# PSeitz/lz4_flex

Measured on AMD Instinct MI355X. Metric: MiB/s compress+decompress round trip, 1 GiB of 64 KiB JSON blocks per GPU (LZ4 block format), higher is better.
Workload: dtype u8

## Files before the change

lz4_flex_amd/csrc/capi.cpp:

```cpp
#include <hip/hip_runtime.h>

#include <algorithm>
#include <cstdio>
#include <cstdlib>
#include <cstring>
#include <mutex>
#include <new>
#include <string>
#include <vector>

#include "../../include/lz4flex_amd.h"
#include "lz4_batch_entry.h"
#include "lz4_ctx.h"
#include "lz4_device.h"
#include "lz4_plan_common.h"

using namespace lz4flex_dev;

static thread_local std::string g_last_error;
static thread_local int g_last_hip = 0;

static int hip_fail(hipError_t e, const char* what) {
    g_last_hip = (int)e;
    g_last_error = std::string(what) + ": " + hipGetErrorString(e);
// ... 278 lines not shown

extern "C" {

const char* lz4flex_version(void) { return "lz4flex-amd 0.3.0 (gfx950)"; }
#ifndef LZ4FLEX_BUILD_ID
#define LZ4FLEX_BUILD_ID "unstamped"
#endif
const char* lz4flex_build_id(void) { return LZ4FLEX_BUILD_ID; }
const char* lz4flex_last_error(void) { return g_last_error.c_str(); }

int lz4flex_device_count(void) {
    int n = 0;
    if (hipGetDeviceCount(&n) != hipSuccess) return 0;
    return n;
}

int lz4flex_ctx_create(lz4flex_ctx** out, int device) {
    if (!out) return -LZ4FLEX_E_INVALID_ARG;
    *out = nullptr;
    int n = 0;
    hipError_t e = hipGetDeviceCount(&n);
    if (e != hipSuccess || n <= 0) {
        g_last_error = "no HIP device available: the MI355X kernels are the only codec in this library";
        return -LZ4FLEX_E_NO_DEVICE;
    }
    if (device < 0) HIP_TRY(hipGetDevice(&device));
    if (device >= n) return -LZ4FLEX_E_INVALID_ARG;
    lz4flex_ctx* c = new (std::nothrow) lz4flex_ctx();
    if (!c) return -LZ4FLEX_E_NOMEM;
    c->device = device;
    c->packed_tile = (int)PACKED_SCAN_TILE;
    if (const char* e = getenv("LZ4FLEX_COMPRESS_MODE")) c->comp_mode = (!strcmp(e, "exact") || !strcmp(e, "1")) ? 1 : (!strcmp(e, "high") || !strcmp(e, "2")) ? 2 : 0;
    if (const char* e = getenv("LZ4FLEX_HIGH_PARSE")) c->comp_parse = (!strcmp(e, "optimal") || !strcmp(e, "1")) ? 1 : 0;
    if (const char* e = getenv("LZ4FLEX_HIGH_DICT")) c->comp_high_dict = !strcmp(e, "1") ? 1 : 0;
    if (const char* e = getenv("LZ4FLEX_HIGH_LINKED")) c->comp_high_linked = !strcmp(e, "1") ? 1 : 0;
    if (const char* e = getenv("LZ4FLEX_SLIDING_WINDOW")) {
        if (!strcmp(e, "0") || !strcmp(e, "1") || !strcmp(e, "2")) c->comp_sliding = e[0] - '0';
        else { g_last_error = "LZ4FLEX_SLIDING_WINDOW must be 0, 1 or 2"; delete c; return -LZ4FLEX_E_INVALID_ARG; }
    }
#ifdef LZ4FLEX_ALL_VARIANTS
    if (const char* e = getenv("LZ4FLEX_COMPRESS_VARIANT")) { const int v = atoi(e); if (v == 1 || v == 3) c->comp_variant = v; }
#endif
    if (const char* e = getenv("LZ4FLEX_DECOMPRESS_VARIANT")) { const int v = atoi(e); if (v == 0 || v == 1 || (v >= 4 && v <= 12 && v != 9)) c->dec_variant = v; }
    {
        DeviceGuard guard(device);
        e = guard.err;
        if (e == hipSuccess) e = hipStreamCreateWithFlags(&c->stream, hipStreamNonBlocking);
        if (e == hipSuccess) {
            int cus = 0;
            e = hipDeviceGetAttribute(&cus, hipDeviceAttributeMultiprocessorCount, device);
            if (e == hipSuccess) {
                c->wave_wgs = 2 * cus;
                e = hipMalloc(&c->wave_ws, compress_wave_workspace_bytes(c->wave_wgs));
            }
        }
        if (e == hipSuccess) e = c->wave.create();
        if (e == hipSuccess) e = hipMalloc((void**)&c->chain_ws, 4u * CHAIN_MAX_BLOCKS);
        if (e == hipSuccess) e = c->chain.create();
        if (e == hipSuccess) e = c->plan.create();
        if (e == hipSuccess) e = c->pcd.create();
        if (e == hipSuccess) e = hipMalloc((void**)&c->pcd_ws, decompress_pcd_pair_ws_bytes());
    }
    if (e != hipSuccess) {
        const int rc = hip_fail(e, "ctx_create");
        lz4flex_ctx_destroy(c);
        return e == hipErrorOutOfMemory ? -LZ4FLEX_E_NOMEM : rc;
    }
    *out = c;
    return 0;
}

void lz4flex_ctx_destroy(lz4flex_ctx* c) {
    if (!c) return;
    c->arena.free();
    if (c->wave_ws) (void)hipFree(c->wave_ws);
    c->wave.destroy();
    if (c->chain_ws) (void)hipFree(c->chain_ws);
    c->chain.destroy();
    if (c->plan_ws) (void)hipFree(c->plan_ws);
    c->plan.destroy();
    if (c->pcd_ws) (void)hipFree(c->pcd_ws);
    c->pcd.destroy();
    if (c->wave_prof) (void)hipFree(c->wave_prof);
    for (void* p : c->many_ws) if (p) (void)hipFree(p);
    c->pin.free();
    c->pay.free();
    if (c->stream) (void)hipStreamDestroy(c->stream);
    delete c;
}

#ifdef LZ4FLEX_TOOLS
int lz4flex_debug_wave_prof(lz4flex_ctx* c, int enable, unsigned long long* vals) {
    if (!c) return -LZ4FLEX_E_INVALID_ARG;
    if (vals && c->wave_prof) {
        HIP_TRY(hipDeviceSynchronize());
        HIP_TRY(hipMemcpy(vals, c->wave_prof, 256, hipMemcpyDeviceToHost));
    }
    if (enable) {
        if (!c->wave_prof) HIP_TRY(hipMalloc((void**)&c->wave_prof, 256));
        HIP_TRY(hipMemset(c->wave_prof, 0, 256));
    } else if (c->wave_prof) {
        (void)hipFree(c->wave_prof);
        c->wave_prof = nullptr;
    }
    return 0;
}
// ... 46 lines not shown
     }, false},
    {"compress_lanes", &lz4flex_ctx::comp_lanes, [](int v) { return v == 8 || v == 16; }, false},
    {"size_scan_serial", &lz4flex_ctx::size_serial, is_flag, false},
    {"filter_bytewise", &lz4flex_ctx::filter_bytewise, is_flag, false},
    {"fit_serial", &lz4flex_ctx::fit_serial, is_flag, false},
    {"compress_shared_dict", &lz4flex_ctx::comp_shared, is_flag, false},
    {"decompress_shared_dict", &lz4flex_ctx::dec_shared, is_flag, false},
    {"decompress_partial", &lz4flex_ctx::dec_partial, is_flag, false},
    {"frame_range_pass_bytes", &lz4flex_ctx::range_pass_bytes, [](int v) { return v >= 1; }, false},
    {"frame_range_checksums", &lz4flex_ctx::range_checksums, is_flag, false},
    {"packed_scan_tile", &lz4flex_ctx::packed_tile, read_only, false},
    {"compress_workgroups", &lz4flex_ctx::wave_wgs, read_only, false},
    {"debug_chain_giveup", &lz4flex_ctx::chain_giveup, is_count, true},
    {"debug_exact_dict_piece", &lz4flex_ctx::exact_dict_piece, is_count, true},
    {"debug_fail_next_batch", &lz4flex_ctx::fail_next_batch, is_count, true},
    {"debug_fit_first_pass", &lz4flex_ctx::fit_first_pass, is_flag, true},
};
const Setting* find_setting(const char* key) {
    for (const Setting& s : SETTINGS) if (!strcmp(key, s.key)) return &s;
    return nullptr;
}

bool key_allowed(const char* key) {
    if (strncmp(key, "debug_", 6) != 0) return true;
    const char* e = getenv("LZ4FLEX_TEST_HOOKS");
    return e && !strcmp(e, "1");
}

int list_index(const char* index) { return index[0] < '0' || index[0] > '9' ? -1 : atoi(index); }

int shared_dict_items(lz4flex_ctx* c) {
    if (!c->shared_counted || !c->wave_ws) return 0;
    DeviceGuard guard(c->device);
    HIP_TRY(guard.err);
    uint32_t v = 0;
    hipError_t e = hipDeviceSynchronize();
    if (e == hipSuccess) e = hipMemcpy(&v, compress_wave_shared_counter(c->wave_ws, c->wave_wgs), 4, hipMemcpyDeviceToHost);
    if (e != hipSuccess) return hip_fail(e, "debug_shared_dict_items");
    return (int)std::min<uint32_t>(v, 0x7FFFFFFFu);
}

int dict_set_items(lz4flex_ctx* c) {
    std::lock_guard<std::mutex> lock(g_sets_mu);
    if (!c->set_counted || std::find(g_live_sets.begin(), g_live_sets.end(), c->set_counted) == g_live_sets.end()) return 0;
    DeviceGuard guard(c->device);
    HIP_TRY(guard.err);
    uint32_t v = 0;
    hipError_t e = hipDeviceSynchronize();
    if (e == hipSuccess) e = hipMemcpy(&v, c->set_counted->counter, 4, hipMemcpyDeviceToHost);
    if (e != hipSuccess) return hip_fail(e, "debug_dict_set_items");
    return (int)std::min<uint32_t>(v, 0x7FFFFFFFu);
}

}

extern "C" {

int lz4flex_set_tuning(lz4flex_ctx* c, const char* key, int value) {
    if (!key) return -LZ4FLEX_E_INVALID_ARG;
    const Setting* st = find_setting(key);
    if (!st || !key_allowed(key)) return -LZ4FLEX_E_INVALID_ARG;
    if (!c) { const int rc = default_ctx(&c); if (rc) return rc; }
    if (!st->takes(value)) return -LZ4FLEX_E_INVALID_ARG;
    c->*(st->field) = value;
    return 0;
}

int lz4flex_get_tuning(lz4flex_ctx* c, const char* key) {
    if (!key) return -LZ4FLEX_E_INVALID_ARG;
    if (!strncmp(key, "dispatch_threshold_", 19)) {
        const int i = list_index(key + 19);
        return i >= 0 && i < (int)(sizeof DISPATCH_THRESHOLDS / sizeof DISPATCH_THRESHOLDS[0]) ? (int)DISPATCH_THRESHOLDS[i] : -LZ4FLEX_E_INVALID_ARG;
    }
    if (!strncmp(key, "decoder_config_", 15)) {
        const int v = decoder_config(list_index(key + 15), TOOLS_BUILD);
        return v >= 0 ? v : -LZ4FLEX_E_INVALID_ARG;
    }
    const bool set_items = !strcmp(key, "debug_dict_set_items");
    const bool items = set_items || !strcmp(key, "debug_shared_dict_items");
    const Setting* st = items ? nullptr : find_setting(key);
    if ((!items && !st) || !key_allowed(key)) return -LZ4FLEX_E_INVALID_ARG;
    if (!c) { const int rc = default_ctx(&c); if (rc) return rc; }
    if (items) return set_items ? dict_set_items(c) : shared_dict_items(c);
    return st->set_only ? -LZ4FLEX_E_INVALID_ARG : c->*(st->field);
}

int lz4flex_abi_version(void) { return 8; }

size_t lz4flex_get_maximum_output_size(size_t input_len) {
    return 16 + 4 + (size_t)((uint64_t)input_len * 110 / 100);
}

}

namespace {

struct Span {
    uint64_t lo = ~0ull, hi = 0;
    void add(uint64_t off, uint64_t len) { lo = std::min<uint64_t>(lo, off); hi = std::max<uint64_t>(hi, off + len); }
    Span closed() const { return lo > hi ? Span{0, 0} : *this; }
    size_t bytes() const { return (size_t)(hi - lo); }
};
Span span_of(const uint64_t* off, const uint32_t* len, uint32_t n) {
    Span s;
    for (uint32_t i = 0; i < n; i++) s.add(off[i], len[i]);
    return s.closed();
}

bool host_big(const uint32_t* len, uint32_t n, bool compress) {
    const uint32_t limit = compress ? 65536u : 131072u;
    bool big = false;
    for (uint32_t i = 0; i < n; i++) big |= len[i] > limit;
    return big;
}

void copy_results(const BatchCall& b, const uint32_t* r_len, const int32_t* r_st, const uint64_t* r_det) {
    memcpy(b.out_len, r_len, 4ull * b.n);
    memcpy(b.status, r_st, 4ull * b.n);
    if (!b.detail) return;
    if (b.compress) memset(b.detail, 0, 16ull * b.n);
    else memcpy(b.detail, r_det, 16ull * b.n);
}

template <class SrcOff>
void scatter_good(uint8_t* out_base, const uint64_t* out_off, const uint32_t* len, const int32_t* st, uint32_t n, const uint8_t* src, SrcOff src_off,
                  uint64_t limit = ~0ull) {
    for (uint32_t i = 0; i < n; i++)
        if ((!st || st[i] == 0) && len[i] && (uint64_t)src_off(i) + len[i] <= limit) memcpy(out_base + out_off[i], src + src_off(i), len[i]);
}

}

static constexpr uint32_t SMALL_BATCH_BLOCKS = 8u;
static constexpr size_t SMALL_BATCH_BYTES = 4u << 20;
static int run_host_small(lz4flex_ctx* c, const BatchCall& b) {
    const uint32_t n = b.n;
// ... 1418 lines not shown
```

lz4_flex_amd/csrc/lz4_compress_wave.hip:

```cpp
#include <hip/hip_runtime.h>
#include <stdint.h>

#include "lz4_device.h"

namespace lz4flex_dev {
namespace wave {

typedef __attribute__((address_space(3))) uint8_t lds_u8;
typedef __attribute__((address_space(3))) uint16_t lds_u16;
typedef __attribute__((address_space(3))) uint32_t lds_u32;
typedef uint32_t u32x4 __attribute__((ext_vector_type(4)));
typedef __attribute__((address_space(1))) uint8_t g_u8;
typedef __attribute__((address_space(1))) u32x4 g_u32x4;
typedef uint32_t u32x2 __attribute__((ext_vector_type(2)));
typedef __attribute__((address_space(1))) u32x2 g_u32x2;
typedef __attribute__((address_space(1))) uint32_t g_u32;
typedef __attribute__((address_space(1))) int32_t g_i32;

constexpr uint32_t WINDOW = 65536u;
#ifndef LZ4W_WORKERS
#define LZ4W_WORKERS 11
#endif
constexpr uint32_t WORKERS = LZ4W_WORKERS;
constexpr uint32_t GROUPS = WINDOW / 512u;
// ... 5 lines not shown
    if (WORKERS == 8u) {
        constexpr uint32_t lo[9] = {0u, 16u, 33u, 50u, 67u, 82u, 98u, 113u, 128u};
        return 512u * lo[w < 8u ? w : 8u];
    }
    return 512u * ((GROUPS * w) / WORKERS);
}
__host__ __device__ constexpr uint32_t seg_longest() {
    uint32_t m = 0u;
    for (uint32_t w = 0u; w < WORKERS; ++w) m = seg_lo(w + 1u) - seg_lo(w) > m ? seg_lo(w + 1u) - seg_lo(w) : m;
    return m;
}
constexpr uint32_t SEG = seg_longest();
constexpr uint32_t HIST = WINDOW / 2u;
__device__ __forceinline__ uint32_t seg_start(uint32_t j, uint32_t skip, uint32_t send) {
    if (send == 0u) return seg_lo(j) > skip ? seg_lo(j) : skip;
    if (j == 0u) return skip;
    if (j >= WORKERS) return send;
    const uint32_t span = send > skip ? send - skip : 0u;
    const uint32_t v = (skip + span * (seg_lo(j) / 512u) / 128u) & ~511u;
    return v > skip ? v : skip;
}

constexpr uint32_t CAP = 1024u;
constexpr uint32_t SKIPD = 64u;
constexpr uint32_t CARRY_SLOTS = 16u;
constexpr uint32_t CARRY_DWORDS = CARRY_SLOTS * 16u;
constexpr uint32_t CARRY_SPINS = 1u << 18;
constexpr uint32_t LONGK = 84u;
constexpr uint32_t NEARP = 20u;
constexpr uint32_t LONGN = 8u;
constexpr uint32_t HBITS = 12u;
constexpr uint32_t THREADS = 64u * (WORKERS + 1u);
#ifndef LZ4W_RING_SLOTS
#define LZ4W_RING_SLOTS 1
#endif
constexpr uint32_t RING_SLOTS = LZ4W_RING_SLOTS;
constexpr uint32_t TMP_OFF = 16u;
constexpr uint32_t CMP_OFF = TMP_OFF + 256u;
constexpr uint32_t WORKER_LDS = CMP_OFF + 256u;
constexpr uint32_t CHUNK = 1024u;
constexpr uint32_t CHUNK_SLOT = CHUNK + 16u;
constexpr uint32_t IDX_DEPTH = 4u;
constexpr uint32_t L_WIN = 0u;
constexpr uint32_t L_TAB = WINDOW + 64u;
constexpr uint32_t L_STG = L_TAB + (2u << HBITS);
constexpr uint32_t L_RING = L_STG + WORKERS * WORKER_LDS;
constexpr uint32_t L_META = L_RING + RING_SLOTS * CHUNK_SLOT;
constexpr uint32_t M_RUN = 5u * WORKERS + 8u;
constexpr uint32_t M_TICKET = M_RUN + 2u;
constexpr uint32_t M_REC = M_TICKET + 1u;
constexpr uint32_t REC_SEG = 7u;
constexpr uint32_t REC_UNI = REC_SEG * WORKERS;
constexpr uint32_t REC_WORDS = REC_UNI + 18u;
constexpr uint32_t META_WORDS = M_REC + 2u * REC_WORDS;
constexpr uint32_t LDS_BYTES = L_META + ((META_WORDS * 4u + 63u) & ~63u);
static_assert(LDS_BYTES <= 81920u, "two workgroups per CU");
static_assert(WORKERS >= 1u && WORKERS <= 15u && seg_lo(WORKERS) == WINDOW, "segments tile the window");
constexpr uint32_t SLOT_BYTES = 2u * WINDOW;
constexpr uint32_t BODY_STRIDE = (SEG + SEG / 128u + 255u) / 256u * 256u + 256u;
constexpr uint32_t BODY_SET = WORKERS * BODY_STRIDE;
constexpr uint32_t WS_BYTES = 2u * SLOT_BYTES + 2u * BODY_SET;
static_assert(WS_BYTES % 256u == 0u, "workspace slots stay 256 B aligned");
constexpr uint32_t STAGE_BYTES = WINDOW + 256u;
constexpr uint32_t STAGE_READ = WINDOW + 64u;

struct SegMeta {
    uint32_t has;
    uint32_t first_lit;
    uint32_t first_ml;
    uint32_t trail;
    uint32_t body_len;
};
struct BlkCarry { uint32_t out_pos, pend; };

__device__ __forceinline__ uint32_t dpp_wave_shr1(uint32_t v, uint32_t lane0) {
    return (uint32_t)__builtin_amdgcn_update_dpp((int)lane0, (int)v, 0x138, 0xf, 0xf, false);
}
__device__ __forceinline__ uint32_t dpp_wave_shl1(uint32_t v, uint32_t lane63) {
    return (uint32_t)__builtin_amdgcn_update_dpp((int)lane63, (int)v, 0x130, 0xf, 0xf, false);
}
#define LZ4W_DPP(v, ctrl, rmask) ((uint32_t)__builtin_amdgcn_update_dpp(0, (int)(v), (ctrl), (rmask), 0xf, false))
__device__ __forceinline__ uint32_t wave_incl_max(uint32_t v) {
    uint32_t t;
    t = LZ4W_DPP(v, 0x111, 0xf); v = v > t ? v : t;
    t = LZ4W_DPP(v, 0x112, 0xf); v = v > t ? v : t;
    t = LZ4W_DPP(v, 0x114, 0xf); v = v > t ? v : t;
    t = LZ4W_DPP(v, 0x118, 0xf); v = v > t ? v : t;
    t = LZ4W_DPP(v, 0x142, 0xa); v = v > t ? v : t;
    t = LZ4W_DPP(v, 0x143, 0xc); v = v > t ? v : t;
    return v;
}
__device__ __forceinline__ uint32_t wave_incl_add(uint32_t v) {
    v += LZ4W_DPP(v, 0x111, 0xf);
    v += LZ4W_DPP(v, 0x112, 0xf);
    v += LZ4W_DPP(v, 0x114, 0xf);
    v += LZ4W_DPP(v, 0x118, 0xf);
    v += LZ4W_DPP(v, 0x142, 0xa);
    v += LZ4W_DPP(v, 0x143, 0xc);
    return v;
}
__device__ __forceinline__ uint32_t rdlane(uint32_t v, uint32_t l) { return (uint32_t)__builtin_amdgcn_readlane((int)v, (int)l); }
__device__ __forceinline__ uint32_t uni(uint32_t v) { return (uint32_t)__builtin_amdgcn_readfirstlane((int)v); }
__device__ __forceinline__ uint64_t ld64l(const lds_u8* p) { uint64_t v; __builtin_memcpy(&v, (const void*)p, 8); return v; }
__device__ __forceinline__ uint32_t umin3(uint32_t a, uint32_t b, uint32_t c) { const uint32_t t = a < b ? a : b; return t < c ? t : c; }
__device__ __forceinline__ uint32_t ctz64(uint64_t x) { return (uint32_t)__builtin_ctzll(x); }
__device__ __forceinline__ uint32_t len_ext_bytes(uint32_t v) { return v >= 15u ? (v - 15u) / 255u + 1u : 0u; }

// ... 184 lines not shown
#endif
#define LZ4W_ONE_CHUNK(N, CC, J)                                                                    \
        {                                                                                           \
            lds_u8* sl = lds + L_RING + ((J) & (RING_SLOTS - 1u)) * CHUNK_SLOT;                                    \
            chunk_wait<N>(q[J]);                                                                    \
            __builtin_memcpy((void*)(sl + 16u * lane), &q[J].main, 16);                             \
            __builtin_memcpy((void*)(sl + CHUNK), &q[J].extra, 4);    \
            const uint32_t cn = (CC) + IDX_DEPTH;                                                   \
            chunk_issue(q[J], gwin, cn < last ? cn : last, lane);                                   \
            index_chunk<true>(sl + lane4, tab, cand_lane, (CC), act_n, lane);                       \
        }
        static_assert(IDX_DEPTH == 4u, "the wait counts below are for four chunks in flight");
        uint32_t c = c0;
        if (n_main - c0 >= IDX_DEPTH) {
            LZ4W_ONE_CHUNK(6, c0, 0)
            LZ4W_ONE_CHUNK(10, c0 + 1u, 1)
            LZ4W_ONE_CHUNK(14, c0 + 2u, 2)
            LZ4W_ONE_CHUNK(18, c0 + 3u, 3)
            c = c0 + IDX_DEPTH;
        }
        for (; c + IDX_DEPTH <= n_main; c += IDX_DEPTH) {
            LZ4W_ONE_CHUNK(22, c, 0)
            LZ4W_ONE_CHUNK(22, c + 1u, 1)
            LZ4W_ONE_CHUNK(22, c + 2u, 2)
            LZ4W_ONE_CHUNK(22, c + 3u, 3)
        }
#undef LZ4W_ONE_CHUNK
        chunk_wait<0>(q[0]); chunk_wait<0>(q[1]); chunk_wait<0>(q[2]); chunk_wait<0>(q[3]);
        for (uint32_t j = 0; c < n_main; ++c, ++j) {
            lds_u8* sl = lds + L_RING + (j & (RING_SLOTS - 1u)) * CHUNK_SLOT;
            const ChunkRegs r = j == 0u ? q[0] : (j == 1u ? q[1] : q[2]);
            __builtin_memcpy((void*)(sl + 16u * lane), &r.main, 16);
            __builtin_memcpy((void*)(sl + CHUNK), &r.extra, 4);
            index_chunk<true>(sl + lane4, tab, cand_lane, c, act_n, lane);
        }
    }
    for (uint32_t c = n_main; c < nchunks; ++c) {
        lds_u8* sl = lds + L_RING;
        const uint32_t base = c * CHUNK;
        for (uint32_t i = lane; i < (CHUNK + 16u) / 16u; i += 64u) {
            const uint32_t o = base + 16u * i;
            u32x4 v = {0u, 0u, 0u, 0u};
            if (o + 16u <= rd_n) __builtin_memcpy(&v, (const void*)(gwin + o), 16);
            __builtin_memcpy((void*)(sl + 16u * i), &v, 16);
        }
        const uint32_t part = rd_n > base ? ((rd_n - base) & ~15u) : 0u;
        if (part < CHUNK + 16u && lane < 16u) {
            const uint32_t o = base + part + lane;
            if (part + lane < CHUNK + 16u) sl[part + lane] = o < rd_n ? gwin[o] : (uint8_t)0;
        }
        index_chunk<false>(sl + lane4, tab, cand_lane, c, act_n, lane);
    }
    return 0u;
}

__device__ __forceinline__ u32x4 tail16(const g_u8* __restrict__ tail, uint32_t o, uint32_t h) {
    u32x4 v = {0u, 0u, 0u, 0u};
    if (o + 16u <= h) __builtin_memcpy(&v, (const void*)(tail + o), 16);
    else if (o < h) {
        uint32_t wd[4] = {0u, 0u, 0u, 0u};
#pragma unroll
        for (uint32_t k = 0; k < 16u; ++k)
            if (o + k < h) wd[k >> 2] |= (uint32_t)tail[o + k] << (8u * (k & 3u));
        v = u32x4{wd[0], wd[1], wd[2], wd[3]};
    }
    return v;
}
__device__ __forceinline__ void digest_body(const uint8_t* __restrict__ dict, uint32_t dict_len, uint8_t* __restrict__ digest,
                                            uint8_t* __restrict__ cand_scratch, lds_u8* lds) {
    const uint32_t lane = threadIdx.x;
    const uint32_t h = dict_len < HIST ? dict_len : HIST, hs = digest_hs(h);
    const g_u8* __restrict__ tail = (const g_u8*)dict + (dict_len - h);
    g_u8* __restrict__ dg = (g_u8*)digest;
    for (uint32_t o = 16u * lane; o < HIST + 256u; o += 1024u) {
        const u32x4 v = tail16(tail, o, h);
        __builtin_memcpy((void*)(dg + DG_TAIL + o), &v, 16);
    }
    const uint32_t splat = h != 0u ? (uint32_t)tail[0] * 0x01010101u : 0u;
    uint32_t acc = 0u;
    for (uint32_t o = 16u * lane; o < hs; o += 1024u) {
        const u32x4 v = tail16(tail, o, h);
        acc |= (v.x ^ splat) | (v.y ^ splat) | (v.z ^ splat) | (v.w ^ splat);
    }
    const uint32_t same = (hs != 0u && __builtin_amdgcn_ballot_w64(acc != 0u) == 0ull) ? 1u : 0u;
    lds_u16* tab = (lds_u16*)lds;
    lds_u8* sl = lds + (2u << HBITS);
    for (uint32_t i = lane; i < (2u << HBITS) / 4u; i += 64u) ((lds_u32*)lds)[i] = 0u;
    for (uint32_t c = 0; c < hs / CHUNK; ++c) {
        for (uint32_t i = lane; i < (CHUNK + 16u) / 16u; i += 64u) {
            const u32x4 v = tail16(tail, c * CHUNK + 16u * i, h);
            __builtin_memcpy((void*)(sl + 16u * i), &v, 16);
        }
        index_chunk<true>(sl + (lane & ~3u), tab, (g_u8*)cand_scratch + 8u * lane, c, hs, lane);
    }
#pragma unroll
    for (uint32_t j = 0; j < 8u; ++j) {
        u32x4 v;
        __builtin_memcpy(&v, (const void*)(lds + 1024u * j + 16u * lane), 16);
        __builtin_memcpy((void*)(dg + DG_TAB + 1024u * j + 16u * lane), &v, 16);
    }
    if (lane == 0u) {
        g_u32* hd = reinterpret_cast<g_u32*>(dg + DG_HDR);
        hd[0] = same; hd[1] = splat; hd[2] = 0u;
    }
}
__global__ void __launch_bounds__(64) lz4_shared_digest_kernel(const uint8_t* __restrict__ dict, uint32_t dict_len, uint8_t* __restrict__ digest,
// ... 860 lines not shown
    item_load(a, it);
}
template <class A>
__device__ __forceinline__ void item_next_block(const A& a, Item& it, int32_t redo) {
    if (it.win + 1u < it.nwin) { it.win += 1u; return; }
    it.blk += gridDim.x;
    item_seek(a, it, redo);
}
template <class A>
__device__ __forceinline__ void item_draw(const A& a, uint32_t* wctr, uint32_t b0, uint32_t& ob, uint32_t& ow) {
    const uint32_t n = a.n;
    uint32_t b = b0;
    const uint32_t tries = n < 8u ? n : 8u;
    for (uint32_t t = 0; t < tries; ++t) {
        Item q;
        q.blk = b;
        item_load(a, q);
        const uint32_t w = atomicAdd(wctr + b, 1u);
        if (w < q.nwin) { ob = b; ow = w; return; }
        b = b + 1u == n ? 0u : b + 1u;
    }
    ob = n; ow = 0u;
}

struct RunGeom { uint32_t ok, ms, me; };
__device__ __forceinline__ RunGeom run_geom(const Item& t) {
    RunGeom g;
    const uint32_t base = win_base(t), wl = win_len(t), skip = win_skip(t);
    g.ms = skip > 1u ? skip : 1u;
    uint32_t me = t.len >= 5u + base ? t.len - 5u - base : 0u;
    me = me < wl ? me : wl;
    g.me = me < 65535u ? me : 65535u;
    const uint32_t act_abs = t.len >= 12u ? t.len - 11u : 0u;
#ifdef LZ4W_NO_RUN_WINDOWS
    g.ok = 0u;
#else
    g.ok = (wl >= RUN_MIN && !t.skip && base + g.ms < act_abs && g.me >= g.ms + 4u) ? 1u : 0u;
#endif
    return g;
}

__device__ __forceinline__ const uint8_t* item_digest(const WaveArgs& a, const Item&) { return a.digest; }
__device__ __forceinline__ uint32_t item_hs(const WaveArgs& a, const Item&) { return a.shared_hs; }
__device__ __forceinline__ uint32_t* item_counter(const WaveArgs& a) { return (uint32_t*)(a.digest + DG_HDR) + 2; }
__device__ __forceinline__ const DictSetRec* set_rec(const SetArgs& a, const Item& t) { return uni_gptr<const DictSetRec>(a.set.table) + uni(t.did); }
__device__ __forceinline__ const uint8_t* item_digest(const SetArgs& a, const Item& t) { return uni_gptr<const uint8_t>(set_rec(a, t)->digest); }
__device__ __forceinline__ uint32_t item_hs(const SetArgs& a, const Item& t) { return a.set.use != 0u ? uni(set_rec(a, t)->hs) : 0u; }
__device__ __forceinline__ uint32_t* item_counter(const SetArgs& a) { return a.set.counter; }
__device__ __forceinline__ uint32_t keep_tag(const WaveArgs& a, const Item&) { return a.shared_keep != 0u ? 1u : 0u; }
__device__ __forceinline__ bool keep_hit(const WaveArgs&, const Item&, uint32_t kept) { return kept != 0u; }
__device__ __forceinline__ uint32_t keep_tag(const SetArgs& a, const Item& t) { return a.set.use != 0u ? t.did + 1u : 0u; }
__device__ __forceinline__ bool keep_hit(const SetArgs&, const Item& t, uint32_t kept) { return kept == t.did + 1u; }

constexpr uint32_t PROF_RESOLVE = 27u;
constexpr uint32_t PROF_IDX_RESOLVE = 28u;
template <class A>
__device__ __forceinline__ void wave_body(const A& a, uint8_t* __restrict__ ws, uint32_t* __restrict__ carry,
                                          unsigned long long* __restrict__ prof, const int32_t redo, const uint32_t carry_spins) {
    extern __shared__ __attribute__((aligned(16))) uint8_t dyn_lds[];
    lds_u8* lds = (lds_u8*)dyn_lds;
    if ((uint32_t)(uintptr_t)lds != 0u) {
        for (uint32_t b = blockIdx.x * THREADS + threadIdx.x; b < a.n; b += gridDim.x * THREADS) { a.out_len[b] = 0u; a.status[b] = 66; }
        return;
    }
    const uint32_t lane = threadIdx.x & 63u;
    const uint32_t w = uni(threadIdx.x >> 6);
#ifdef LZ4W_EXP_IDX_PRIO
    if (w == WORKERS) __builtin_amdgcn_s_setprio(LZ4W_EXP_IDX_PRIO);
#endif
    uint8_t* my_ws = ws + (size_t)blockIdx.x * WS_BYTES;
    uint8_t* slots = my_ws;
    uint8_t* bodies = my_ws + 2u * SLOT_BYTES;
    uint8_t* stg = a.stage + (size_t)blockIdx.x * STAGE_BYTES;

    const bool wmode = carry != nullptr;
    lds_u32* giq = (lds_u32*)(lds + L_META) + 5u * WORKERS + 4u;
    uint32_t* wctr = wmode ? carry + CARRY_DWORDS * (size_t)a.n : nullptr;
    Item it, ix;
    lds_u32* meta = (lds_u32*)(lds + L_META);
    if (threadIdx.x == 0u) {
        meta[M_TICKET] = 0u;
        meta[M_REC + REC_UNI + RU_COUNT] = 0u;
        meta[M_REC + REC_WORDS + REC_UNI + RU_COUNT] = 0u;
    }
    if (wmode) {
        if (threadIdx.x == 0u) {
            uint32_t b = a.n, wn = 0u;
            item_draw(a, wctr, blockIdx.x % a.n, b, wn);
            giq[0] = b; giq[1] = wn;
        }
        __syncthreads();
        it.blk = giq[0];
        item_load(a, it);
        it.win = giq[1];
        ix.blk = a.n;
        item_load(a, ix);
    } else {
        it.blk = blockIdx.x;
        item_seek(a, it, redo);
        ix = it;
        item_next_block(a, ix, redo);
    }
    if (it.blk >= a.n) return;
    uint32_t k = 0u;

    lds_u32* run_flag = (lds_u32*)(lds + L_META) + M_RUN;
// ... 1 lines not shown
    auto do_stage = [&](const Item& t) {
        const uint32_t base = win_base(t);
        const uint32_t nrd = win_rd(t);
        if constexpr (HAS_DIGEST<A>) {
            const uint32_t from = (t.win == 0u && keep_hit(a, t, tail_kept)) ? (t.hist & ~15u) : 0u;
            stage_window(item_digest(a, t) + DG_TAIL, a.in_base + t.in_off, base + from, nrd - from, t.hist, stg + from, lane);
            tail_kept = t.win == 0u ? keep_tag(a, t) : 0u;
            return;
        } else {
        const uint8_t* tail = a.dict_base + a.dict_off[t.blk] + (a.dict_len[t.blk] - t.hist);
        stage_window(tail, a.in_base + t.in_off, base, nrd, t.hist, stg, lane);
        }
    };
    auto do_index = [&](const Item& t, uint32_t slot, bool stage) {
        if (t.skip) { if (lane == 0u) run_flag[slot] = 0u; return; }
        if (t.dct && stage) do_stage(t);
        const uint32_t base = win_base(t), wl = win_len(t);
        const uint32_t act_abs = t.len >= 12u ? t.len - 11u : 0u;
        const uint32_t act_n = act_abs > base ? (act_abs - base < wl ? act_abs - base : wl) : 0u;
        const RunGeom rg = run_geom(t);
        if constexpr (HAS_DIGEST<A>) {
            const uint32_t hs = (IS_SHARED<A> || t.dct != 0u) ? item_hs(a, t) : 0u;
            if (t.win == 0u && hs != 0u && act_n >= hs) {
                const uint32_t run = index_window<true>(win_src(a, t, stg), wl, act_n, win_rd(t), slots + (size_t)slot * SLOT_BYTES, lds, lane, rg.ok,
                                                        DigestRef<true>{item_digest(a, t), hs});
                if (redo == 0 && lane == 0u)
                    __hip_atomic_fetch_add(item_counter(a), 1u, __ATOMIC_RELAXED, __HIP_MEMORY_SCOPE_AGENT);
                if (lane == 0u) run_flag[slot] = run;
                return;
            }
        }
        const uint32_t run = index_window<false>(win_src(a, t, stg), wl, act_n, win_rd(t), slots + (size_t)slot * SLOT_BYTES, lds, lane, rg.ok, DigestRef<false>{});
        if (lane == 0u) run_flag[slot] = run;
    };
    auto do_load = [&](const Item& t) {
        if (t.skip) return;
        load_window(win_src(a, t, stg), win_len(t), win_rd(t), lds, threadIdx.x);
    };

    uint64_t t_prev = prof ? __builtin_readcyclecounter() : 0ull;
    uint64_t t_acc[8] = {0ull, 0ull, 0ull, 0ull, 0ull, 0ull, 0ull, 0ull};
    auto tick = [&](uint32_t slot) {
        if (prof) {
            const uint64_t t = __builtin_readcyclecounter();
#pragma unroll
            for (uint32_t i = 0; i < 8u; ++i) t_acc[i] += i == slot ? t - t_prev : 0ull;
            t_prev = t;
        }
    };
    if (it.dct && !it.skip) {
        if (w == WORKERS) do_stage(it);
        __syncthreads();
    }
    if (w == WORKERS) { do_index(it, 0u, false); tick(0u); }
    else { do_load(it); tick(5u); }
    __syncthreads();
    tick(w == WORKERS ? 1u : 6u);
    if (wmode) {
        if (threadIdx.x == 0u) {
            uint32_t b2 = a.n, w2 = 0u;
            item_draw(a, wctr, it.blk, b2, w2);
            giq[2] = b2; giq[3] = w2;
        }
        __syncthreads();
        ix.blk = giq[2];
        item_load(a, ix);
        ix.win = giq[3];
        __syncthreads();
    }
    for (;;) {
        const uint32_t wl = win_len(it);
        const bool last_win = it.win + 1u == it.nwin;
        const uint32_t crec = M_REC + ((k + 1u) & 1u) * REC_WORDS;
        auto draw = [&]() -> uint32_t {
            uint32_t t = 0u;
            if (lane == 0u) t = __hip_atomic_fetch_add(meta + M_TICKET, 1u, __ATOMIC_RELAXED, __HIP_MEMORY_SCOPE_WORKGROUP);
            return uni(t);
        };
        if (w == WORKERS) {
            if (ix.blk < a.n) do_index(ix, (k + 1u) & 1u, true);
#ifdef LZ4W_EXP_IDX_TICKET
            const uint32_t icnt = uni(meta[crec + REC_UNI + RU_COUNT]);
            const uint32_t itk = icnt != 0u ? draw() : icnt;
            if (itk < icnt) {
                __builtin_amdgcn_fence(__ATOMIC_ACQUIRE, "workgroup");
                copy_segment(lds, crec, icnt - 1u - itk, bodies + (size_t)((k + 1u) & 1u) * BODY_SET, lane);
            }
#endif
        } else if (!it.skip) {
            const uint32_t base = win_base(it), skip = win_skip(it);
            uint32_t s0 = seg_start(w, skip, win_send(it));
            uint32_t s1 = seg_start(w + 1u, skip, win_send(it));
            s0 = s0 < wl ? s0 : wl;
            s1 = s1 < wl ? s1 : wl;
            const uint32_t act_abs = it.len >= 12u ? it.len - 11u : 0u;
            const uint32_t mfl_end = act_abs > base ? act_abs - base : 0u;
            uint32_t mend = it.len >= 5u ? it.len - 5u : 0u;
            mend = mend > base ? mend - base : 0u;
            mend = mend < s1 ? mend : s1;
            mend = mend < 65535u ? mend : 65535u;
            if (run_flag[k & 1u] != 0u) {
                const RunGeom rg = run_geom(it);
                lds_u32* mp = (lds_u32*)(lds + L_META) + 5u * w;
                if (w == 0u) {
                    emit_generic(bodies + (size_t)(k & 1u) * BODY_SET, 0u, 0u, 0u, 1u, rg.me - rg.ms, 1u, lane);
                    if (lane == 0u) { mp[0] = 1u; mp[1] = rg.ms - skip; mp[2] = rg.me - rg.ms; mp[3] = wl - rg.me; mp[4] = 2u + len_ext_bytes(rg.me - rg.ms - 4u); }
                } else if (lane == 0u) {
                    mp[0] = 0u; mp[1] = 0u; mp[2] = 0u; mp[3] = 0u; mp[4] = 0u;
// ... 96 lines not shown
    static_cast<CompressArgs&>(r) = no_dicts(a);
    r.flags = nullptr;
    r.shared_dict = sh.dict; r.shared_len = sh.len; r.shared_hs = sh.hs; r.shared_keep = sh.keep; r.digest = sh.digest;
    return r;
}
__device__ __forceinline__ SetArgs only_set(const CompressArgs& a, const DictSetArgs& st) {
    SetArgs r;
    static_cast<CompressArgs&>(r) = no_dicts(a);
    r.flags = nullptr;
    r.set = st;
    return r;
}
__global__ void __launch_bounds__(THREADS) __attribute__((amdgpu_waves_per_eu(6, 6))) lz4_compress_wave_kernel(const CompressArgs a, uint8_t* __restrict__ ws,
                                                                    uint32_t* __restrict__ carry, unsigned long long* __restrict__ prof, uint32_t carry_spins) {
    wave_body(no_dicts(a), ws, carry, prof, 0, carry_spins);
}
__global__ void __launch_bounds__(THREADS) __attribute__((amdgpu_waves_per_eu(6, 6))) lz4_compress_wave_redo_kernel(const CompressArgs a, uint8_t* __restrict__ ws,
                                                                                                                     int32_t redo) {
    wave_body(no_dicts(a), ws, nullptr, nullptr, redo, CARRY_SPINS);
}
__global__ void __launch_bounds__(THREADS) __attribute__((amdgpu_waves_per_eu(6, 6))) lz4_compress_wave_dict_kernel(const CompressArgs a, uint8_t* __restrict__ ws,
                                                                    uint32_t* __restrict__ carry, unsigned long long* __restrict__ prof, uint32_t carry_spins) {
    wave_body(a, ws, carry, prof, 0, carry_spins);
}
__global__ void __launch_bounds__(THREADS) __attribute__((amdgpu_waves_per_eu(6, 6))) lz4_compress_wave_dict_redo_kernel(const CompressArgs a, uint8_t* __restrict__ ws,
                                                                                                                          int32_t redo) {
    wave_body(a, ws, nullptr, nullptr, redo, CARRY_SPINS);
}
__global__ void __launch_bounds__(THREADS) __attribute__((amdgpu_waves_per_eu(6, 6))) lz4_compress_wave_shared_kernel(const CompressArgs a, const SharedDictArgs sh,
                                                                    uint8_t* __restrict__ ws, uint32_t* __restrict__ carry, unsigned long long* __restrict__ prof, uint32_t carry_spins) {
    wave_body(only_shared(a, sh), ws, carry, prof, 0, carry_spins);
}
__global__ void __launch_bounds__(THREADS) __attribute__((amdgpu_waves_per_eu(6, 6))) lz4_compress_wave_shared_redo_kernel(const CompressArgs a, const SharedDictArgs sh,
                                                                                                                            uint8_t* __restrict__ ws, int32_t redo) {
    wave_body(only_shared(a, sh), ws, nullptr, nullptr, redo, CARRY_SPINS);
}
__global__ void __launch_bounds__(THREADS) __attribute__((amdgpu_waves_per_eu(6, 6))) lz4_wave_set_kernel(const CompressArgs a, const DictSetArgs st,
                                                                    uint8_t* __restrict__ ws, uint32_t* __restrict__ carry, unsigned long long* __restrict__ prof, uint32_t carry_spins) {
    wave_body(only_set(a, st), ws, carry, prof, 0, carry_spins);
}
__global__ void __launch_bounds__(THREADS) __attribute__((amdgpu_waves_per_eu(6, 6))) lz4_wave_set_redo_kernel(const CompressArgs a, const DictSetArgs st,
                                                                                                                         uint8_t* __restrict__ ws, int32_t redo) {
    wave_body(only_set(a, st), ws, nullptr, nullptr, redo, CARRY_SPINS);
}

}

static size_t wave_stage_at(int n_workgroups) { return ((size_t)n_workgroups * (wave::WS_BYTES + wave::CARRY_DWORDS * 4u + 4u) + 255u) & ~(size_t)255u; }
static size_t wave_digest_at(int n_workgroups) { return wave_stage_at(n_workgroups) + (size_t)n_workgroups * wave::STAGE_BYTES; }
size_t compress_wave_workspace_bytes(int n_workgroups) { return wave_digest_at(n_workgroups) + wave::DIGEST_BYTES; }
const uint32_t* compress_wave_shared_counter(const void* workspace, int n_workgroups) {
    return (const uint32_t*)((const uint8_t*)workspace + wave_digest_at(n_workgroups) + wave::DG_HDR) + 2;
}

size_t compress_wave_digest_bytes() { return wave::DIGEST_BYTES; }
uint32_t compress_wave_digest_hs(uint32_t h) { return wave::digest_hs(h); }
size_t compress_wave_digest_scratch_bytes() { return wave::DIGEST_SCRATCH; }
hipError_t launch_dict_set_digests(const DictSetRec* table, uint32_t k, uint8_t* cand_scratch, hipStream_t s) {
    if (k == 0u) return hipSuccess;
    hipLaunchKernelGGL(wave::lz4_set_digest_kernel, dim3(k), dim3(64), (2u << wave::HBITS) + wave::CHUNK_SLOT, s, table, cand_scratch);
    return hipGetLastError();
}

hipError_t launch_compress_wave(const CompressArgs& a, void* workspace, int n_workgroups, hipStream_t s, unsigned long long* prof, bool carry_wait,
                                const SharedDictArgs* shared_dict, const DictSetArgs* dict_set) {
    if (a.n == 0u) return hipSuccess;
    if (!workspace || n_workgroups <= 0) return hipErrorInvalidValue;
    static unsigned long long have = 0ull;
    int dev = 0;
    (void)hipGetDevice(&dev);
    const unsigned long long bit = 1ull << (dev & 63);
    if (!(have & bit)) {
        for (const void* k : {reinterpret_cast<const void*>(wave::lz4_compress_wave_kernel), reinterpret_cast<const void*>(wave::lz4_compress_wave_redo_kernel),
                              reinterpret_cast<const void*>(wave::lz4_compress_wave_dict_kernel),
                              reinterpret_cast<const void*>(wave::lz4_compress_wave_dict_redo_kernel),
                              reinterpret_cast<const void*>(wave::lz4_compress_wave_shared_kernel),
                              reinterpret_cast<const void*>(wave::lz4_compress_wave_shared_redo_kernel),
                              reinterpret_cast<const void*>(wave::lz4_wave_set_kernel),
                              reinterpret_cast<const void*>(wave::lz4_wave_set_redo_kernel)}) {
            const hipError_t e = hipFuncSetAttribute(k, hipFuncAttributeMaxDynamicSharedMemorySize, (int)wave::LDS_BYTES);
            if (e != hipSuccess) return e;
        }
        have |= bit;
    }
    uint32_t* carry = nullptr;
    if (a.n < (uint32_t)n_workgroups) {
        carry = (uint32_t*)((uint8_t*)workspace + (size_t)n_workgroups * wave::WS_BYTES);
        const hipError_t e = hipMemsetAsync(carry, 0, (size_t)a.n * (wave::CARRY_DWORDS * 4u + 4u), s);
        if (e != hipSuccess) return e;
    }
    CompressArgs as = a;
    as.stage = (uint8_t*)workspace + wave_stage_at(n_workgroups);
    const bool dicts = as.dict_base != nullptr && as.dict_off != nullptr && as.dict_len != nullptr;
    const bool shared = shared_dict != nullptr && shared_dict->dict != nullptr && shared_dict->len != 0u;
    const uint32_t spins = carry_wait ? wave::CARRY_SPINS : 1u;
    SharedDictArgs sh{};
    if (dict_set != nullptr) {
        if (shared || dicts || dict_set->table == nullptr || dict_set->dict_id == nullptr || dict_set->counter == nullptr) return hipErrorInvalidValue;
        hipLaunchKernelGGL(wave::lz4_wave_set_kernel, dim3((uint32_t)n_workgroups), dim3(wave::THREADS), wave::LDS_BYTES, s, as, *dict_set,
                           (uint8_t*)workspace, carry, prof, spins);
    } else if (shared) {
        sh = *shared_dict;
        sh.digest = (uint8_t*)workspace + wave_digest_at(n_workgroups);
        const uint32_t h = sh.len < wave::HIST ? sh.len : wave::HIST;
        sh.hs = sh.use != 0u ? wave::digest_hs(h) : 0u;
        sh.keep = sh.use;
// ... 35 lines not shown
```

lz4_flex_amd/csrc/lz4_device.h:

```cpp
#pragma once
#include <hip/hip_runtime.h>
#include <stdint.h>

#include "lz4_route.h"

#define LZ4FLEX_DEV_E_OUTPUT_TOO_SMALL 1
#define LZ4FLEX_DEV_E_LITERAL_OUT_OF_BOUNDS 2
#define LZ4FLEX_DEV_E_EXPECTED_ANOTHER_BYTE 3
#define LZ4FLEX_DEV_E_OFFSET_ZERO 4
#define LZ4FLEX_DEV_E_OFFSET_OUT_OF_BOUNDS 5
#define LZ4FLEX_DEV_E_UNSUPPORTED 68
#define LZ4FLEX_DEV_E_INVALID_ARG 64

namespace lz4flex_range { struct RangeRec; }

namespace lz4flex_dev {

struct DecompressArgs {
    const uint8_t* in_base;
    const uint64_t* in_off;
    const uint32_t* in_len;
    uint8_t* out_base;
    const uint64_t* out_off;
    const uint32_t* out_cap;
// ... 94 lines not shown
        r.refused = r.len != 0u && a.flags != nullptr && a.flags[b] != 0u;
    }
    return r;
}
template <typename Rec>
__host__ __device__ inline Rec dict_chain_record(uint64_t in_off, uint32_t in_len, uint64_t dict_end, uint64_t dict_len) {
    const uint32_t kept = dict_len > 65536u ? 65536u : (uint32_t)dict_len;
    return Rec{in_off, dict_end - kept, in_len, 0u, kept, kept, 0u, (dict_len + in_len < 65535u ? 1u : 0u) | 2u};
}

namespace plan { struct BlockPlan; }
struct ReplayArgs {
    const uint8_t* in_base;
    uint8_t* out_base;
    const plan::BlockPlan* plans;
    const uint32_t* words;
    uint32_t n;
    uint32_t max_turns;
};
hipError_t launch_replay(const ReplayArgs& a, hipStream_t s);
struct PlanArgs {
    const uint8_t* in_base;
    const uint64_t* in_off;
    const uint32_t* in_len;
    const uint64_t* out_off;
    const uint32_t* out_cap;
    plan::BlockPlan* plans;
    uint32_t* words;
    uint32_t* out_len;
    int32_t* status;
    uint32_t n;
    uint32_t slot_words;
    int32_t redo_code;
};
size_t plan_slot_words();
hipError_t launch_plan(const PlanArgs& a, hipStream_t s);

hipError_t launch_decompress(const DecompressArgs& a, int lanes_per_block, hipStream_t s);
hipError_t launch_decompress(const DecompressArgs& a, const DictSource& d, bool partial, int lanes_per_block, hipStream_t s);
hipError_t launch_decompress_seq(const DecompressArgs& a, const DictSource& d, bool partial, int32_t redo_code, hipStream_t s);
inline bool decode_form_ok(const DecompressArgs& a, const DictSource& d, bool partial) {
    if (!d.has_set && d.shared == nullptr && !partial) return true;
    if (a.dict_base != nullptr || a.out_pos != nullptr || a.chain_done != nullptr) return false;
    if (d.has_set) return d.set.table != nullptr && d.set.dict_id != nullptr;
    return d.shared == nullptr || d.shared_len != 0u;
}
hipError_t launch_decompress_chain_redo(const DecompressArgs& a, hipStream_t s);
hipError_t launch_decompress_split(const DecompressArgs& a, hipStream_t s, int blocks_per_wg = 0);
hipError_t launch_decompress_fused(const DecompressArgs& a, int32_t redo_code, hipStream_t s);
hipError_t launch_decompress_pcd(const DecompressArgs& a, int32_t redo_code, hipStream_t s, int geometry = 0);
hipError_t launch_compress(const CompressArgs& a, int variant, hipStream_t s);
size_t compress_wave_workspace_bytes(int n_workgroups);
const uint32_t* compress_wave_shared_counter(const void* workspace, int n_workgroups);
hipError_t launch_compress_wave(const CompressArgs& a, void* workspace, int n_workgroups, hipStream_t s,
                                unsigned long long* prof = nullptr,
                                bool carry_wait = true,
                                const SharedDictArgs* shared_dict = nullptr,
                                const DictSetArgs* dict_set = nullptr);
size_t compress_high_workspace_bytes(int n_workgroups);
hipError_t launch_compress_high(const CompressArgs& a, void* workspace, size_t workspace_bytes, int max_workgroups, uint32_t depth, uint32_t parse, hipStream_t s);
hipError_t launch_compress_high_dict(const CompressArgs& a, const DictSource& d, bool use_digest, void* workspace, size_t workspace_bytes,
                                     int max_workgroups, uint32_t depth, uint32_t parse, hipStream_t s);
hipError_t launch_compress_high_linked(const CompressArgs& a, void* workspace, size_t workspace_bytes, int max_workgroups, uint32_t depth,
                                       uint32_t parse, hipStream_t s);
size_t compress_wave_digest_bytes();
uint32_t compress_wave_digest_hs(uint32_t h);
size_t compress_wave_digest_scratch_bytes();
hipError_t launch_dict_set_digests(const DictSetRec* table, uint32_t k, uint8_t* cand_scratch, hipStream_t s);

hipError_t launch_compress_chain(const uint8_t* in_base, const void* blocks, const uint32_t* chain_first,
                                 const uint32_t* chain_count, uint32_t n_chains, uint8_t* out_base,
                                 const uint64_t* out_off, const uint32_t* out_cap, uint32_t* out_len, int32_t* status,
                                 uint32_t* tbl_state, hipStream_t s, const uint8_t* dict_base = nullptr);
hipError_t launch_compress_exact(const CompressArgs& a, const DictSource& d, int enc_bits, bool big, void* ws, size_t ws_bytes,
                                 uint32_t max_piece, hipStream_t s);

hipError_t launch_xxh32_batch(const uint8_t* base, const uint64_t* off, const uint32_t* len, uint32_t n, uint32_t seed,
                              uint32_t* out, hipStream_t s);

hipError_t launch_frame_assemble(const uint8_t* src_base, const uint64_t* src_off, const uint32_t* in_len, const uint8_t* comp_base,
                                 const uint64_t* comp_off, const uint32_t* comp_len, uint32_t n, int block_checksums, uint8_t* seg,
                                 uint64_t* seg_off, uint64_t* pay_off, uint32_t* pay_len, uint32_t* sums, hipStream_t s);
hipError_t launch_frame_walk(const uint8_t* f, uint64_t n, uint32_t hdr, uint32_t tail, uint32_t block_size, uint32_t max_blocks, uint64_t* off,
                             uint32_t* len, uint32_t* info, hipStream_t s);
struct ManyStream { uint64_t out_off, out_cap; uint32_t first, count, hdr_len, flags; uint8_t hdr[24]; };
struct ManyFrame { uint64_t off, len; uint32_t hdr_len, block_size, flags, slot, slot_cap, skip; };
hipError_t launch_frame_many_assemble(const ManyStream* st, uint32_t n_streams, const uint8_t* src_base, const uint64_t* src_off, const uint32_t* in_len,
                                      const uint8_t* comp_base, const uint64_t* comp_off, const uint32_t* comp_len, const int32_t* comp_st, uint32_t n_blocks,
                                      int block_checksums, const uint32_t* content_sum, uint8_t* out_base, uint64_t* dst_off, uint64_t* pay_off,
                                      uint32_t* pay_len, uint32_t* sums, uint64_t* frame_len, int32_t* verdict, hipStream_t s);
hipError_t launch_frame_many_heads(const uint8_t* base, const uint64_t* off, const uint64_t* len, uint32_t n, uint8_t* heads, hipStream_t s);
hipError_t launch_frame_many_walk(const uint8_t* base, const ManyFrame* fr, uint32_t n, uint64_t* pay_off, uint32_t* word, uint32_t* info, hipStream_t s);
hipError_t launch_frame_sums_check(const uint8_t* base, const uint64_t* pay_off, const uint32_t* pay_len, const uint32_t* sums, uint32_t n, uint32_t* bad,
                                   hipStream_t s);
hipError_t launch_copy_batch(const uint8_t* src_base, const uint64_t* src_off, const uint32_t* len, uint8_t* dst_base, const uint64_t* dst_off,
                             uint32_t n, hipStream_t s);

constexpr int32_t SIZE_SCAN_REDO = 0x7F000003;
hipError_t launch_size_scan(const uint8_t* in_base, const uint64_t* in_off, const uint32_t* in_len, const uint32_t* history, uint32_t n,
                            uint64_t* out_size, int32_t* status, int serial_only, hipStream_t s);
constexpr int32_t FIT_REDO = 0x7F000004;
struct FitArgs {
    const uint8_t* blk_base; const uint64_t* blk_off; const uint32_t* blk_len;
    const uint8_t* src_base; const uint64_t* src_off; const uint32_t* src_len;
    uint32_t n;
    uint8_t* out_base; const uint64_t* out_off; const uint32_t* out_cap;
// ... 93 lines not shown
```

Before: 224,000.

## Parallelize wave compressor prologue hash-table indexing across multiple wavefronts

Replaces the single-wavefront serial indexing prologue of the wave compressor with a partitioned scheme. Up to eight wavefronts each build a partial hash table over their own chunk range, using scratch space in the LDS window area. The partial tables are then merged as a prefix so each part sees the latest earlier positions, and each part runs the candidate pass over its range. This targets the latency of the serial per-block prologue, at the cost of extra LDS passes, barriers and a per-block uniformity check. It also adds a debug counter, reachable through the tuning API, that reports how many blocks took the parallel path.

```diff
diff --git a/lz4_flex_amd/csrc/capi.cpp b/lz4_flex_amd/csrc/capi.cpp
--- a/lz4_flex_amd/csrc/capi.cpp
+++ b/lz4_flex_amd/csrc/capi.cpp
@@ -354,6 +354,7 @@
             if (e == hipSuccess) {
                 c->wave_wgs = 2 * cus;
                 e = hipMalloc(&c->wave_ws, compress_wave_workspace_bytes(c->wave_wgs));
+                if (e == hipSuccess) e = hipMemset(compress_wave_parts_counter(c->wave_ws, c->wave_wgs), 0, 4);
             }
         }
         if (e == hipSuccess) e = c->wave.create();
@@ -506,6 +507,17 @@
     return (int)std::min<uint32_t>(v, 0x7FFFFFFFu);
 }
 
+int parallel_prologue_items(lz4flex_ctx* c) {
+    if (!c->wave_ws) return 0;
+    DeviceGuard guard(c->device);
+    HIP_TRY(guard.err);
+    uint32_t v = 0;
+    hipError_t e = hipDeviceSynchronize();
+    if (e == hipSuccess) e = hipMemcpy(&v, compress_wave_parts_counter(c->wave_ws, c->wave_wgs), 4, hipMemcpyDeviceToHost);
+    if (e != hipSuccess) return hip_fail(e, "debug_parallel_prologue_items");
+    return (int)(v & 0x7FFFFFFFu);
+}
+
 }
 
 extern "C" {
@@ -531,11 +543,12 @@
         return v >= 0 ? v : -LZ4FLEX_E_INVALID_ARG;
     }
     const bool set_items = !strcmp(key, "debug_dict_set_items");
-    const bool items = set_items || !strcmp(key, "debug_shared_dict_items");
+    const bool par_items = !strcmp(key, "debug_parallel_prologue_items");
+    const bool items = set_items || par_items || !strcmp(key, "debug_shared_dict_items");
     const Setting* st = items ? nullptr : find_setting(key);
     if ((!items && !st) || !key_allowed(key)) return -LZ4FLEX_E_INVALID_ARG;
     if (!c) { const int rc = default_ctx(&c); if (rc) return rc; }
-    if (items) return set_items ? dict_set_items(c) : shared_dict_items(c);
+    if (items) return set_items ? dict_set_items(c) : (par_items ? parallel_prologue_items(c) : shared_dict_items(c));
     return st->set_only ? -LZ4FLEX_E_INVALID_ARG : c->*(st->field);
 }
 
diff --git a/lz4_flex_amd/csrc/lz4_compress_wave.hip b/lz4_flex_amd/csrc/lz4_compress_wave.hip
--- a/lz4_flex_amd/csrc/lz4_compress_wave.hip
+++ b/lz4_flex_amd/csrc/lz4_compress_wave.hip
@@ -81,7 +81,8 @@
 constexpr uint32_t REC_SEG = 7u;
 constexpr uint32_t REC_UNI = REC_SEG * WORKERS;
 constexpr uint32_t REC_WORDS = REC_UNI + 18u;
-constexpr uint32_t META_WORDS = M_REC + 2u * REC_WORDS;
+constexpr uint32_t M_PAR = M_REC + 2u * REC_WORDS;
+constexpr uint32_t META_WORDS = M_PAR + 1u;
 constexpr uint32_t LDS_BYTES = L_META + ((META_WORDS * 4u + 63u) & ~63u);
 static_assert(LDS_BYTES <= 81920u, "two workgroups per CU");
 static_assert(WORKERS >= 1u && WORKERS <= 15u && seg_lo(WORKERS) == WINDOW, "segments tile the window");
@@ -372,6 +373,110 @@
         index_chunk<false>(sl + lane4, tab, cand_lane, c, act_n, lane);
     }
     return 0u;
+}
+
+#ifndef LZ4W_PARTS
+#define LZ4W_PARTS 8
+#endif
+constexpr uint32_t PARTS = LZ4W_PARTS;
+constexpr uint32_t PART_LDS = (2u << HBITS) + CHUNK_SLOT;
+static_assert((PARTS - 1u) * PART_LDS <= WINDOW + 64u && PART_LDS % 16u == 0u, "the parts' tables and chunk slots fit the window area");
+static_assert(PARTS >= 2u && PARTS <= WORKERS + 1u, "a wavefront per part");
+__device__ __forceinline__ uint32_t part_tab_off(uint32_t p) { return p == 0u ? L_TAB : L_WIN + (p - 1u) * PART_LDS; }
+__device__ __forceinline__ uint32_t part_slot_off(uint32_t p) { return p == 0u ? L_RING : L_WIN + (p - 1u) * PART_LDS + (2u << HBITS); }
+__device__ __forceinline__ uint32_t main_chunks(uint32_t wl, uint32_t act_n, uint32_t rd_n) {
+    const uint32_t nchunks = (wl + CHUNK - 1u) / CHUNK;
+    uint32_t n_main = rd_n >= CHUNK + 4u ? (rd_n - 4u) / CHUNK : 0u;
+    n_main = n_main < act_n / CHUNK ? n_main : act_n / CHUNK;
+    return n_main < nchunks ? n_main : nchunks;
+}
+__device__ __forceinline__ void insert_chunk(const lds_u8* lp, lds_u16* tab, uint32_t c, uint32_t lane) {
+#pragma unroll
+    for (uint32_t g8 = 0; g8 < 2u; ++g8) {
+        uint64_t xr[8];
+#pragma unroll
+        for (uint32_t u = 0; u < 8u; ++u)
+            asm volatile("ds_read2_b32 %0, %1 offset0:%2 offset1:%3" : "=v"(xr[u]) : "v"((uint32_t)(uintptr_t)lp), "n"((g8 * 8u + u) * 16u), "n"((g8 * 8u + u) * 16u + 1u) : "memory");
+        asm volatile("s_waitcnt lgkmcnt(0)" : "+v"(xr[0]), "+v"(xr[1]), "+v"(xr[2]), "+v"(xr[3]), "+v"(xr[4]), "+v"(xr[5]), "+v"(xr[6]), "+v"(xr[7]) :: "memory");
+#pragma unroll
+        for (uint32_t u = 0; u < 8u; ++u) {
+            const uint32_t x = __builtin_amdgcn_alignbyte((uint32_t)(xr[u] >> 32), (uint32_t)xr[u], lane);
+            tab[(x * 2654435761u) >> (32u - HBITS)] = (uint16_t)(c * CHUNK + (g8 * 8u + u) * 64u + lane);
+        }
+    }
+}
+template <bool INDEX>
+__device__ __forceinline__ void part_walk(const g_u8* __restrict__ gwin, lds_u8* sl, lds_u16* tab, g_u8* __restrict__ cand_lane, uint32_t c0, uint32_t c1,
+                                          uint32_t act_n, uint32_t lane) {
+    ChunkRegs q;
+    chunk_issue(q, gwin, c0, lane);
+    chunk_wait<0>(q);
+    for (uint32_t c = c0; c < c1; ++c) {
+        __builtin_memcpy((void*)(sl + 16u * lane), &q.main, 16);
+        __builtin_memcpy((void*)(sl + CHUNK), &q.extra, 4);
+        chunk_issue(q, gwin, c + 1u < c1 ? c + 1u : c, lane);
+        if (INDEX) index_chunk<true>(sl + (lane & ~3u), tab, cand_lane, c, act_n, lane);
+        else insert_chunk(sl + (lane & ~3u), tab, c, lane);
+        chunk_wait<INDEX ? 4 : 0>(q);
+    }
+}
+__device__ __attribute__((noinline)) void index_parts(const uint8_t* __restrict__ gwin_, uint32_t wl_, uint32_t act_n_, uint32_t rd_n_,
+                                                      uint8_t* __restrict__ slot_t_, lds_u8* lds, uint32_t w_, uint32_t lane) {
+    const g_u8* __restrict__ gwin = uni_gptr<const g_u8>(gwin_);
+    g_u8* __restrict__ slot_t = uni_gptr<g_u8>(slot_t_);
+    const uint32_t wl = uni(wl_), act_n = uni(act_n_), rd_n = uni(rd_n_), w = uni(w_);
+    const uint32_t n_main = main_chunks(wl, act_n, rd_n);
+    const uint32_t nchunks = (wl + CHUNK - 1u) / CHUNK;
+    const bool mine = w < PARTS;
+    const uint32_t p = mine ? w : 0u;
+    const uint32_t c0 = p * n_main / PARTS, c1 = (p + 1u) * n_main / PARTS;
+    lds_u16* tab = (lds_u16*)(lds + part_tab_off(p));
+    lds_u8* sl = lds + part_slot_off(p);
+    g_u8* cand_lane = slot_t + 8u * lane;
+    if (mine && p + 1u < PARTS) {
+        const u32x4 z = {0u, 0u, 0u, 0u};
+        for (uint32_t i = lane; i < (2u << HBITS) / 16u; i += 64u) __builtin_memcpy((void*)((lds_u8*)tab + 16u * i), &z, 16);
+#ifndef LZ4W_EXP_PARTS_FULL_PASS1
+        part_walk<false>(gwin, sl, tab, cand_lane, c0, c1, act_n, lane);
+#else
+        part_walk<true>(gwin, sl, tab, cand_lane, c0, c1, act_n, lane);
+#endif
+    }
+    __syncthreads();
+    for (uint32_t i = w * 64u + lane; i < (1u << HBITS) / 2u; i += THREADS) {
+        uint32_t t[PARTS - 1u];
+#pragma unroll
+        for (uint32_t j = 0; j + 1u < PARTS; ++j) t[j] = ((const lds_u32*)(lds + part_tab_off(j)))[i];
+        uint32_t s = 0u;
+        ((lds_u32*)(lds + part_tab_off(0u)))[i] = 0u;
+#pragma unroll
+        for (uint32_t j = 1u; j < PARTS; ++j) {
+            const uint32_t x = t[j - 1u];
+            s = ((x & 0xFFFFu) != 0u ? (x & 0xFFFFu) : (s & 0xFFFFu)) | ((x >> 16) != 0u ? (x & 0xFFFF0000u) : (s & 0xFFFF0000u));
+            ((lds_u32*)(lds + part_tab_off(j)))[i] = s;
+        }
+    }
+    __syncthreads();
+    if (mine) {
+        part_walk<true>(gwin, sl, tab, cand_lane, c0, c1, act_n, lane);
+        if (p + 1u == PARTS) {
+            for (uint32_t c = n_main; c < nchunks; ++c) {
+                const uint32_t base = c * CHUNK;
+                for (uint32_t i = lane; i < (CHUNK + 16u) / 16u; i += 64u) {
+                    const uint32_t o = base + 16u * i;
+                    u32x4 v = {0u, 0u, 0u, 0u};
+                    if (o + 16u <= rd_n) __builtin_memcpy(&v, (const void*)(gwin + o), 16);
+                    __builtin_memcpy((void*)(sl + 16u * i), &v, 16);
+                }
+                const uint32_t part = rd_n > base ? ((rd_n - base) & ~15u) : 0u;
+                if (part < CHUNK + 16u && lane < 16u) {
+                    const uint32_t o = base + part + lane;
+                    if (part + lane < CHUNK + 16u) sl[part + lane] = o < rd_n ? gwin[o] : (uint8_t)0;
+                }
+                index_chunk<false>(sl + (lane & ~3u), tab, cand_lane, c, act_n, lane);
+            }
+        }
+    }
 }
 
 __device__ __forceinline__ u32x4 tail16(const g_u8* __restrict__ tail, uint32_t o, uint32_t h) {
@@ -1338,6 +1443,8 @@
 __device__ __forceinline__ uint32_t keep_tag(const SetArgs& a, const Item& t) { return a.set.use != 0u ? t.did + 1u : 0u; }
 __device__ __forceinline__ bool keep_hit(const SetArgs&, const Item& t, uint32_t kept) { return kept == t.did + 1u; }
 
+constexpr uint32_t DG_PARTS = 3u;
+__device__ __forceinline__ uint32_t* parts_counter(uint8_t* stage) { return (uint32_t*)(stage + (size_t)gridDim.x * STAGE_BYTES + DG_HDR) + DG_PARTS; }
 constexpr uint32_t PROF_RESOLVE = 27u;
 constexpr uint32_t PROF_IDX_RESOLVE = 28u;
 template <class A>
@@ -1445,8 +1552,40 @@
         if (w == WORKERS) do_stage(it);
         __syncthreads();
     }
-    if (w == WORKERS) { do_index(it, 0u, false); tick(0u); }
-    else { do_load(it); tick(5u); }
+    bool par = false;
+#ifndef LZ4W_SERIAL_PROLOGUE
+    if constexpr (!HAS_DIGEST<A>) {
+        const uint32_t base = win_base(it), pwl = win_len(it);
+        const uint32_t act_abs = it.len >= 12u ? it.len - 11u : 0u;
+        const uint32_t act_n = act_abs > base ? (act_abs - base < pwl ? act_abs - base : pwl) : 0u;
+        par = !it.skip && !it.dct && it.hist == 0u && main_chunks(pwl, act_n, win_rd(it)) >= PARTS;
+        if (par) {
+            const uint8_t* gw = win_src(a, it, stg);
+            if (w == 0u) {
+                u32x4 v;
+                __builtin_memcpy(&v, (const void*)(uni_gptr<const g_u8>(gw) + 16u * lane), 16);
+                const uint32_t splat = (v.x & 255u) * 0x01010101u;
+                const uint32_t dif = (v.x ^ splat) | (v.y ^ splat) | (v.z ^ splat) | (v.w ^ splat);
+                const bool varied = __builtin_amdgcn_ballot_w64((dif != 0u) | (splat != uni(splat))) != 0ull;
+                if (lane == 0u) { meta[M_PAR] = varied ? 1u : 0u; run_flag[0] = 0u; }
+            }
+            __syncthreads();
+            par = uni(meta[M_PAR]) != 0u;
+            if (par) {
+                index_parts(gw, pwl, act_n, win_rd(it), slots, lds, w, lane);
+                if (redo == 0 && threadIdx.x == 0u)
+                    __hip_atomic_fetch_add(parts_counter(a.stage), 1u, __ATOMIC_RELAXED, __HIP_MEMORY_SCOPE_AGENT);
+                tick(w == WORKERS ? 0u : 6u);
+                __syncthreads();
+                if (w != WORKERS) { do_load(it); tick(5u); }
+            }
+        }
+    }
+#endif
+    if (!par) {
+        if (w == WORKERS) { do_index(it, 0u, false); tick(0u); }
+        else { do_load(it); tick(5u); }
+    }
     __syncthreads();
     tick(w == WORKERS ? 1u : 6u);
     if (wmode) {
@@ -1649,6 +1788,9 @@
 const uint32_t* compress_wave_shared_counter(const void* workspace, int n_workgroups) {
     return (const uint32_t*)((const uint8_t*)workspace + wave_digest_at(n_workgroups) + wave::DG_HDR) + 2;
 }
+uint32_t* compress_wave_parts_counter(void* workspace, int n_workgroups) {
+    return (uint32_t*)((uint8_t*)workspace + wave_digest_at(n_workgroups) + wave::DG_HDR) + wave::DG_PARTS;
+}
 
 size_t compress_wave_digest_bytes() { return wave::DIGEST_BYTES; }
 uint32_t compress_wave_digest_hs(uint32_t h) { return wave::digest_hs(h); }
diff --git a/lz4_flex_amd/csrc/lz4_device.h b/lz4_flex_amd/csrc/lz4_device.h
--- a/lz4_flex_amd/csrc/lz4_device.h
+++ b/lz4_flex_amd/csrc/lz4_device.h
@@ -170,6 +170,7 @@
 hipError_t launch_compress(const CompressArgs& a, int variant, hipStream_t s);
 size_t compress_wave_workspace_bytes(int n_workgroups);
 const uint32_t* compress_wave_shared_counter(const void* workspace, int n_workgroups);
+uint32_t* compress_wave_parts_counter(void* workspace, int n_workgroups);
 hipError_t launch_compress_wave(const CompressArgs& a, void* workspace, int n_workgroups, hipStream_t s,
                                 unsigned long long* prof = nullptr,
                                 bool carry_wait = true,
```

Result: no change. 225,000, median of 6 (+0.4%).
